# line/Human-Interaction-Generation

Measured on AMD Instinct MI355X. Metric: denoiser-fwd frames/s @ B=64·T=196, higher is better.
Workload: dtype f32; 1 GPU; MotionTransformer forward incl. the per-call cross-attention text side, BASELINE config 2: B=64/GPU T=196 F=150 d=512 L=8 H=8 ff=1024 N=77 Lt=256, linear attention, text embeddings supplied (CLIP stubbed); parallelism=dp1

## Files before the change

human-interaction-generation_amd/csrc/denoiser.hip:

```cpp
#include <stdarg.h>
#include <stdio.h>
#include <string.h>

#include "hig_common.h"
#include "hig_host.h"

static thread_local char g_err[512] = "";
int hig_set_error(int code, const char* fmt, ...) {
  va_list ap;
  va_start(ap, fmt);
  vsnprintf(g_err, sizeof(g_err), fmt, ap);
  va_end(ap);
  return code;
}
extern "C" int hig_last_error(char* buf, int n) {
  if (buf && n > 0) {
    strncpy(buf, g_err, (size_t)n - 1);
    buf[n - 1] = 0;
  }
  return (int)strlen(g_err);
}
extern "C" int hig_version(void) { return 100; }

namespace {
// ... 367 lines not shown
namespace {

constexpr int kMaxTextLayers = 32;
struct SideStream {
  hipStream_t s2 = nullptr;
  hipEvent_t ready = nullptr;
  hipEvent_t done[4] = {nullptr, nullptr, nullptr, nullptr};
  hipStream_t s3 = nullptr;
  hipEvent_t text_done[kMaxTextLayers] = {};
  bool ok = false, failed = false;
};

constexpr int kMaxDev = 16;
SideStream* side_stream_table() {
  static thread_local SideStream tab[kMaxDev];
  return tab;
}

hipEvent_t& layer_event() {
  static thread_local hipEvent_t ev = nullptr;
  return ev;
}

int bwd_overlap_env() {
  static const int v = getenv("HIG_BWD_OVERLAP") ? atoi(getenv("HIG_BWD_OVERLAP")) : -1;
  return v;
}

SideStream* side_stream_for_current_device(hipStream_t caller) {
  if (bwd_overlap_env() == 0) return nullptr;
  SideStream* tab = side_stream_table();
  int dev = 0;
  if (hipGetDevice(&dev) != hipSuccess || dev < 0 || dev >= kMaxDev) return nullptr;
  SideStream& s = tab[dev];
  if (s.failed) return nullptr;
  if (!s.ok) {
    hipStreamCaptureStatus cap = hipStreamCaptureStatusNone;
    if (hipStreamIsCapturing(caller, &cap) != hipSuccess || cap != hipStreamCaptureStatusNone) return nullptr;
    bool good = hipStreamCreateWithFlags(&s.s2, hipStreamNonBlocking) == hipSuccess;
    good = good && hipEventCreateWithFlags(&s.ready, hipEventDisableTiming) == hipSuccess;
    for (int i = 0; i < 4 && good; ++i) good = hipEventCreateWithFlags(&s.done[i], hipEventDisableTiming) == hipSuccess;
    good = good && hipStreamCreateWithFlags(&s.s3, hipStreamNonBlocking) == hipSuccess;
    for (int i = 0; i < kMaxTextLayers && good; ++i) good = hipEventCreateWithFlags(&s.text_done[i], hipEventDisableTiming) == hipSuccess;
    if (!good) {
      s.failed = true;
      return nullptr;
    }
    s.ok = true;
  }
  return &s;
}

}

static int denoiser_fwd_impl(const hig_dims* dims, const void* const* params, const void* const* derived32, const float* x, const int64_t* t,
                             const int64_t* length, const float* xf_proj, const float* xf_out_for_text, const void* textctx, float* out,
                             void* workspace, int training, hig_stream_t stream);
extern "C" int hig_denoiser_fwd(const hig_dims* dims, const void* const* params, const float* x,
                                const int64_t* t, const int64_t* length, const float* xf_proj,
                                const void* textctx, float* out, void* workspace, int training,
                                hig_stream_t stream) {
  return denoiser_fwd_impl(dims, params, nullptr, x, t, length, xf_proj, nullptr, textctx, out, workspace, training, stream);
}
extern "C" int hig_denoiser_fwd_text(const hig_dims* dims, const void* const* params, const float* x, const int64_t* t,
                                     const int64_t* length, const float* xf_proj, const float* xf_out, void* textctx, float* out,
                                     void* workspace, int training, hig_stream_t stream) {
  HIG_REQUIRE(xf_out, "hig_denoiser_fwd_text: null argument");
  return denoiser_fwd_impl(dims, params, nullptr, x, t, length, xf_proj, xf_out, textctx, out, workspace, training, stream);
}
extern "C" int hig_denoiser_fwd_x(const hig_dims* dims, const void* const* params, const void* const* derived32, const float* x,
                                  const int64_t* t, const int64_t* length, const float* xf_proj, const float* xf_out, void* textctx,
                                  float* out, void* workspace, int training, hig_stream_t stream) {
  return denoiser_fwd_impl(dims, params, derived32, x, t, length, xf_proj, xf_out, textctx, out, workspace, training, stream);
}
static int denoiser_fwd_impl(const hig_dims* dims, const void* const* params, const void* const* derived32, const float* x, const int64_t* t,
                             const int64_t* length, const float* xf_proj, const float* xf_out_for_text, const void* textctx, float* out,
                             void* workspace, int training, hig_stream_t stream) {
  Dims D;
  HIG_TRY(check_dims(dims, D));
  HIG_REQUIRE(params && x && t && xf_proj && textctx && out && workspace, "hig_denoiser_fwd: null argument");
  HIG_REQUIRE(!D.bf16, "hig_denoiser_fwd: bf16 storage goes through hig_denoiser_fwd_bf16");
  const FwdLayout w = fwd_layout(D, training);
  const TextLayout tl = text_layout(D, training);
  float* ws = static_cast<float*>(workspace);
  const float* tc = static_cast<const float*>(textctx);
  hipStream_t st = hig_stream(stream);
  const int d = D.d, E = D.E;
  const int64_t M = D.M;
  const int64_t ss_ld = (int64_t)D.nsty * D.L * 2 * d;
  const int Bp = D.B / 2;

  HIG_TRY(hig_zero_async(ws + w.gtail, HIG_GEMM_TAIL_CNT_BYTES, st));
  const TailScratchScope tail_scope(ws + w.gtail);

  hipEvent_t* text_ev = nullptr;
  struct TextJoin {
    hipStream_t s3 = nullptr, st = nullptr;
    hipEvent_t ev = nullptr;
    bool armed = false;
    void arm(hipStream_t s3_, hipEvent_t ev_, hipStream_t st_) { s3 = s3_; ev = ev_; st = st_; armed = true; }
    ~TextJoin() {
      if (!armed) return;
      (void)hipEventRecord(ev, s3);
      (void)hipStreamWaitEvent(st, ev, 0);
    }
  } text_join;
  if (xf_out_for_text) {
    static const int text_fork = getenv("HIG_TEXT_FORK") ? atoi(getenv("HIG_TEXT_FORK")) : 1;
    SideStream* ts = (text_fork && D.L <= kMaxTextLayers && !text_batched(D, derived32, training)) ? side_stream_for_current_device(st) : nullptr;
    if (ts) {
      hipStreamCaptureStatus cap = hipStreamCaptureStatusNone;
      if (hipStreamIsCapturing(st, &cap) != hipSuccess || cap != hipStreamCaptureStatusNone) ts = nullptr;
    }
    if (ts) {
      HIG_TRY(hig_zero_async(ws + w.gtail3, HIG_GEMM_TAIL_CNT_BYTES, st));
      if (hipEventRecord(ts->ready, st) != hipSuccess || hipStreamWaitEvent(ts->s3, ts->ready, 0) != hipSuccess)
        return hig_set_error(HIG_EHIP, "text fork failed");
      hig_gemm_set_tail_scratch(ws + w.gtail3, HIG_GEMM_TAIL_BYTES);
      const int rc = text_context_impl(D, params, derived32, xf_out_for_text, const_cast<void*>(textctx), training, ts->s3, ts->text_done);
      hig_gemm_set_tail_scratch(ws + w.gtail, HIG_GEMM_TAIL_BYTES);
      text_join.arm(ts->s3, ts->text_done[0], st);
      if (rc != HIG_OK) return rc;
      text_ev = ts->text_done;
    } else {
      HIG_TRY(text_context_impl(D, params, derived32, xf_out_for_text, const_cast<void*>(textctx), training, st, nullptr));
    }
  }
  HIG_TRY(hig_timestep_embedding(t, D.B, d, ws + w.te, stream));
  float* few_scratch = ws + w.layer0;
  const int64_t few_floats = w.total - w.layer0;
  HIG_TRY(hig_gemm_few_rows(G(ws + w.te, d, 0, P(params, HIG_P_TE0_W), d, 0, ws + w.te_h, E, D.B, E, d)
                                .epi(HIG_EPI_BIAS, P(params, HIG_P_TE0_B)).prec(D.prec).g, few_scratch, few_floats, st));
  HIG_TRY(hig_gemm_few_rows(G(ws + w.te_h, E, 0, P(params, HIG_P_TE2_W), E, 0, ws + w.emb, E, D.B, E, E)
                                .silu(0).epi(HIG_EPI_BIAS_RES, P(params, HIG_P_TE2_B)).res(xf_proj, E).prec(D.prec).g,
                            few_scratch, few_floats, st));
  HIG_TRY(hig_gemm_few_rows(G(ws + w.emb, E, 0, P(params, HIG_P_STY_EMB_W), E, 0, ws + w.ss, ss_ld, D.B, ss_ld, E)
                                .silu(0).epi(HIG_EPI_BIAS, P(params, HIG_P_STY_EMB_B)).prec(D.prec).g, few_scratch, few_floats,
                            st));
  {
    G ge(x, D.F, 0, P(params, HIG_P_JOINT_W), D.F, 0, ws + w.h0, d, M, d, D.F);
    ge.epi(HIG_EPI_BIAS_POS, P(params, HIG_P_JOINT_B)).pos(P(params, HIG_P_SEQ_EMB), d, D.T).prec(D.prec);
    ge.g.pos_shift = D.two ? 1 : 0;
    HIG_TRY(hig_gemm_launch(ge.g, 1, nullptr, st));
  }
  const int64_t* len_partner = nullptr;
  if (D.two) {
    HIG_TRY(hig_gemm_launch(G(x, (int64_t)D.T * D.F, 0, P(params, HIG_P_JOINT2_W), 4, 0, ws + w.h0, (int64_t)D.T * d,
                              D.B, d, 4).epi(HIG_EPI_BIAS, P(params, HIG_P_JOINT2_B)).g, 1, nullptr, st));
    int64_t* lp = reinterpret_cast<int64_t*>(ws + w.lenp);
    hipLaunchKernelGGL(swap_halves_i64_kernel, dim3((D.B + 255) / 256), dim3(256), 0, st, length, D.B, (int64_t)D.T, lp);
    HIG_CHECK_LAUNCH();
    len_partner = lp;
  }
  constexpr int fuse_env = 0;
  const bool fuse_apply = fuse_env && !training && !D.full && (D.H == 4 || D.H == 8) && (D.hd == 64 || D.hd == 128);
  static const int fold_env = getenv("HIG_LNFOLD32") ? atoi(getenv("HIG_LNFOLD32")) : 1;
  const bool fold32 = fold_env && derived32 && !training && d % 128 == 0 && d <= 1024;
  const Derived d32 = derived32_table(D, derived32);
  int layer_rc = HIG_OK;
  auto layer = [&](int l, const float* hin_full, int b0, int nb, hipStream_t s, float* cscr) -> const float* {
    hig_stream_t hs = reinterpret_cast<hig_stream_t>(s);
    float* lb = ws + w.layer0 + w.lstride * l;
    const int64_t r0 = (int64_t)b0 * D.T, Mh = (int64_t)nb * D.T;
    const int64_t aoff = (int64_t)b0 * D.H * D.hd * D.hd;
    const float* ssl = ws + w.ss + (int64_t)(D.nsty * l) * 2 * d + (int64_t)b0 * ss_ld;
    const float* ss_ffn = ssl + (int64_t)(D.nsty - 1) * 2 * d;
    const int64_t* len = length ? length + b0 : nullptr;
    const float* hin = hin_full + r0 * d;
    auto R = [&](int64_t off, int64_t ld) { return lb + off + r0 * ld; };
    auto fail = [&](int rc) -> const float* { layer_rc = rc; return nullptr; };
#define HIG_L(expr) do { const int rc_ = (expr); if (rc_ != HIG_OK) return fail(rc_); } while (0)
    const int np = d >> 6;
    float* lnst = ws + w.lnstats + r0 * np * 2;
    auto folded = [&](int k) { return fold32 && d32.layer(l, HIG_D32_SA_QKV_W + 3 * k) != nullptr; };
    auto ln_proj = [&](int k, bool have_stats, const float* hrows, int norm_w, int norm_b, int lin_w, int lin_b, float* xn, float* st,
                       float* outp, int ncols) -> int {
      if (have_stats && folded(k)) {
        G gf(hrows, d, 0, d32.layer<float>(l, HIG_D32_SA_QKV_W + 3 * k), d, 0, outp, ncols, Mh, ncols, d);
        gf.epi(HIG_EPI_BIAS, d32.layer<float>(l, HIG_D32_SA_QKV_B + 3 * k)).prec(D.prec);
        gf.g.row_stats_in = lnst;
        gf.g.ln_colsum = d32.layer<float>(l, HIG_D32_SA_QKV_COLSUM + 3 * k);
        return hig_gemm_launch(gf.g, 1, nullptr, s);
      }
      HIG_TRY(hig_layernorm(hrows, d, Mh, d, PL(params, l, norm_w), PL(params, l, norm_b), xn, d, st, hs));
      return hig_gemm_launch(G(xn, d, 0, PL(params, l, lin_w), d, 0, outp, ncols, Mh, ncols, d)
                                 .epi(HIG_EPI_BIAS, PL(params, l, lin_b)).prec(D.prec).g, 1, nullptr, s);
    };
    HIG_L(ln_proj(0, l > 0 && folded(0), hin, HIG_L_SA_NORM_W, HIG_L_SA_NORM_B, HIG_L_SA_QKV_W, HIG_L_SA_QKV_B, R(w.xn1, d), R(w.st1, 2),
                  R(w.qkv, 3 * d), 3 * d));
    if (D.full) {
      HIG_L(hig_fullattn_fwd(R(w.qkv, 3 * d), 3 * d, R(w.qkv, 3 * d) + d, R(w.qkv, 3 * d) + 2 * d, 3 * d, nb, D.T, D.T, D.H, D.hd,
                             len, R(w.y1, d), d, lb + w.lse1 + (int64_t)b0 * D.H * D.T, hs));
    } else {
      HIG_L(hig_linattn_ctx(R(w.qkv, 3 * d) + d, R(w.qkv, 3 * d) + 2 * d, 3 * d, nb, D.T, D.H, D.hd, len,
                            lb + w.A1 + aoff, lb + w.kst1 + (int64_t)b0 * d * 2, cscr, hs));
      if (fuse_apply)
        HIG_L(hig_linattn_apply_sty(R(w.qkv, 3 * d), 3 * d, lb + w.A1 + aoff, PL(params, l, HIG_L_SA_STY_NORM_W),
                                    PL(params, l, HIG_L_SA_STY_NORM_B), ssl, ss_ld, d, R(w.a1, d), d, nb, D.T, D.H, D.hd, hs));
      else
        HIG_L(hig_linattn_apply(R(w.qkv, 3 * d), 3 * d, lb + w.A1 + aoff, R(w.y1, d), d, nb, D.T, D.H, D.hd, hs));
    }
    if (!fuse_apply)
      HIG_L(hig_ln_mod_silu(R(w.y1, d), d, Mh, d, PL(params, l, HIG_L_SA_STY_NORM_W), PL(params, l, HIG_L_SA_STY_NORM_B),
                            ssl, ss_ld, d, D.T, R(w.a1, d), d, R(w.st2, 2), hs));
    {
      G gs(R(w.a1, d), d, 0, PL(params, l, HIG_L_SA_STY_OUT_W), d, 0, R(w.h1, d), d, Mh, d, d);
      gs.epi(HIG_EPI_BIAS_RES, PL(params, l, HIG_L_SA_STY_OUT_B)).res(hin, d).prec(D.prec);
      if (folded(1)) gs.g.row_stats_out = lnst;
      HIG_L(hig_gemm_launch(gs.g, 1, nullptr, s));
    }
    HIG_L(ln_proj(1, folded(1), R(w.h1, d), HIG_L_CA_NORM_W, HIG_L_CA_NORM_B, HIG_L_CA_Q_W, HIG_L_CA_Q_B, R(w.xn2, d), R(w.st3, 2),
                  R(w.qc, d), d));
    const float* Acl = tc + tl.layer0 + tl.lstride * l + tl.Ac + aoff;
    if (text_ev && hipStreamWaitEvent(s, text_ev[l], 0) != hipSuccess) return fail(hig_set_error(HIG_EHIP, "text join failed"));
    if (D.full) {
      const float* kvl = tc + tl.kv + tl.kv_stride * l + (int64_t)b0 * D.N * 2 * d;
      HIG_L(hig_fullattn_fwd(R(w.qc, d), d, kvl, kvl + d, 2 * d, nb, D.T, D.N, D.H, D.hd, nullptr, R(w.y2, d), d,
                             lb + w.lse2 + (int64_t)b0 * D.H * D.T, hs));
    } else {
      if (fuse_apply)
        HIG_L(hig_linattn_apply_sty(R(w.qc, d), d, Acl, PL(params, l, HIG_L_CA_STY_NORM_W),
                                    PL(params, l, HIG_L_CA_STY_NORM_B), ssl + 2 * d, ss_ld, d, R(w.a2, d), d, nb, D.T, D.H, D.hd, hs));
      else
        HIG_L(hig_linattn_apply(R(w.qc, d), d, Acl, R(w.y2, d), d, nb, D.T, D.H, D.hd, hs));
    }
    if (!fuse_apply)
      HIG_L(hig_ln_mod_silu(R(w.y2, d), d, Mh, d, PL(params, l, HIG_L_CA_STY_NORM_W), PL(params, l, HIG_L_CA_STY_NORM_B),
                            ssl + 2 * d, ss_ld, d, D.T, R(w.a2, d), d, R(w.st4, 2), hs));
    HIG_L(hig_gemm_launch(G(R(w.a2, d), d, 0, PL(params, l, HIG_L_CA_STY_OUT_W), d, 0, R(w.h2, d), d, Mh, d, d)
                              .epi(HIG_EPI_BIAS_RES, PL(params, l, HIG_L_CA_STY_OUT_B)).res(R(w.h1, d), d).prec(D.prec).g, 1, nullptr, s));
    const float* hffn = R(w.h2, d);
    int64_t hffn_off = w.h2;
    if (D.two == 1) {
      HIG_L(hig_layernorm(lb + w.h2, d, M, d, PL(params, l, HIG_L_INT_NORM_W), PL(params, l, HIG_L_INT_NORM_B),
                          lb + w.xn3, d, lb + w.st6, hs));
      HIG_L(hig_gemm_launch(G(lb + w.xn3, d, 0, PL(params, l, HIG_L_INT_QKV_W), d, 0, lb + w.iqkv, 3 * d, M, 3 * d, d)
                                .epi(HIG_EPI_BIAS, PL(params, l, HIG_L_INT_QKV_B)).prec(D.prec).g, 1, nullptr, s));
      HIG_L(hig_linattn_ctx(lb + w.iqkv + d, lb + w.iqkv + 2 * d, 3 * d, D.B, D.T, D.H, D.hd, len_partner,
                            lb + w.Ai, lb + w.ksti, cscr, hs));
      const int64_t halfA = (int64_t)Bp * D.H * D.hd * D.hd, halfM = (int64_t)Bp * D.T;
      HIG_L(hig_linattn_apply(lb + w.iqkv, 3 * d, lb + w.Ai + halfA, lb + w.y4, d, Bp, D.T, D.H, D.hd, hs));
      HIG_L(hig_linattn_apply(lb + w.iqkv + halfM * 3 * d, 3 * d, lb + w.Ai, lb + w.y4 + halfM * d, d, Bp, D.T, D.H,
                              D.hd, hs));
      HIG_L(hig_ln_mod_silu(lb + w.y4, d, M, d, PL(params, l, HIG_L_INT_STY_NORM_W), PL(params, l, HIG_L_INT_STY_NORM_B),
                            ssl + 4 * d, ss_ld, d, D.T, lb + w.a4, d, lb + w.st7, hs));
      HIG_L(hig_gemm_launch(G(lb + w.a4, d, 0, PL(params, l, HIG_L_INT_STY_OUT_W), d, 0, lb + w.h2b, d, M, d, d)
                                .epi(HIG_EPI_BIAS_RES, PL(params, l, HIG_L_INT_STY_OUT_B)).res(lb + w.h2, d).prec(D.prec).g,
                            1, nullptr, s));
      hffn = lb + w.h2b;
      hffn_off = w.h2b;
    }
    (void)hffn_off;
    HIG_L(hig_gemm_launch(G(hffn, d, 0, PL(params, l, HIG_L_FFN_W1), d, 0, R(w.f1, D.ff), D.ff, Mh, D.ff, d)
                              .epi(HIG_EPI_BIAS_GELU, PL(params, l, HIG_L_FFN_B1))
                              .aux(training ? R(w.z1, D.ff) : nullptr, D.ff).prec(D.prec).g, 1, nullptr, s));
    HIG_L(hig_gemm_launch(G(R(w.f1, D.ff), D.ff, 0, PL(params, l, HIG_L_FFN_W2), D.ff, 0, R(w.y3, d), d, Mh, d, D.ff)
                              .epi(HIG_EPI_BIAS, PL(params, l, HIG_L_FFN_B2)).prec(D.prec).g, 1, nullptr, s));
    HIG_L(hig_ln_mod_silu(R(w.y3, d), d, Mh, d, PL(params, l, HIG_L_FFN_STY_NORM_W), PL(params, l, HIG_L_FFN_STY_NORM_B),
                          ss_ffn, ss_ld, d, D.T, R(w.a3, d), d, R(w.st5, 2), hs));
    {
      G gs(R(w.a3, d), d, 0, PL(params, l, HIG_L_FFN_STY_OUT_W), d, 0, R(w.h3, d), d, Mh, d, d);
      gs.epi(HIG_EPI_BIAS_RES, PL(params, l, HIG_L_FFN_STY_OUT_B)).res(hffn, d).prec(D.prec);
      if (fold32 && l + 1 < D.L && d32.layer(l + 1, HIG_D32_SA_QKV_W) != nullptr) gs.g.row_stats_out = lnst;
      HIG_L(hig_gemm_launch(gs.g, 1, nullptr, s));
    }
#undef HIG_L
    return lb + w.h3;
  };
  auto out_proj = [&](const float* hin_full, int b0, int nb, hipStream_t s) -> int {
    const int64_t r0 = (int64_t)b0 * D.T;
    return hig_gemm_launch(G(hin_full + r0 * d, d, 0, P(params, HIG_P_OUT_W), d, 0, out + r0 * D.F, D.F, (int64_t)nb * D.T, D.F, d)
                               .epi(HIG_EPI_BIAS, P(params, HIG_P_OUT_B)).prec(D.prec).g, 1, nullptr, s);
  };

  static const int split_knob = getenv("HIG_FWD_SPLIT") ? atoi(getenv("HIG_FWD_SPLIT")) : -1;
  const int split_env = split_knob >= 0 ? split_knob : ((D.prec == HIG_PREC_F32 && hig_gemm_wsp32_active()) ? 0 : 1);
  SideStream* side = (split_env && !D.two && D.B >= 16 && M >= 8192) ? side_stream_for_current_device(st) : nullptr;
  if (side) {
    hipStreamCaptureStatus cap = hipStreamCaptureStatusNone;
    if (hipStreamIsCapturing(st, &cap) != hipSuccess || cap != hipStreamCaptureStatusNone) side = nullptr;
  }
  const float* hin = ws + w.h0;
  if (side) {
    const int nbA = D.B / 2, nbB = D.B - nbA;
    HIG_TRY(hig_zero_async(ws + w.gtail2, HIG_GEMM_TAIL_CNT_BYTES, st));
    if (hipEventRecord(side->ready, st) != hipSuccess || hipStreamWaitEvent(side->s2, side->ready, 0) != hipSuccess)
      return hig_set_error(HIG_EHIP, "forward fork failed");
    int rc = HIG_OK;
    for (int l = 0; l < D.L && rc == HIG_OK; ++l) {
      hig_gemm_set_tail_scratch(ws + w.gtail, HIG_GEMM_TAIL_BYTES);
      const float* ha = layer(l, hin, 0, nbA, st, ws + w.cscr);
      const float* hb = nullptr;
      if (ha) {
        hig_gemm_set_tail_scratch(ws + w.gtail2, HIG_GEMM_TAIL_BYTES);
        hb = layer(l, hin, nbA, nbB, side->s2, ws + w.cscr2);
      }
      if (!ha || !hb) rc = layer_rc != HIG_OK ? layer_rc : HIG_EHIP;
      else hin = ha;
    }
    if (rc == HIG_OK) {
      hig_gemm_set_tail_scratch(ws + w.gtail, HIG_GEMM_TAIL_BYTES);
      rc = out_proj(hin, 0, nbA, st);
    }
    if (rc == HIG_OK) {
      hig_gemm_set_tail_scratch(ws + w.gtail2, HIG_GEMM_TAIL_BYTES);
      rc = out_proj(hin, nbA, nbB, side->s2);
    }
    hig_gemm_set_tail_scratch(ws + w.gtail, HIG_GEMM_TAIL_BYTES);
// ... 1507 lines not shown
```

human-interaction-generation_amd/csrc/linattn.hip:

```cpp
#include <stdlib.h>

#include "hig_common.h"

int hig_chip_cus();

namespace {

constexpr int CH = 64;

template <int HD> struct Patch {
  static constexpr int PC = HD >= 128 ? 8 : HD >= 64 ? 4 : HD >= 32 ? 2 : 1;
  static constexpr int PL = PC;
  static constexpr int TL = HD / PL;
};

template <int HD>
__global__ __launch_bounds__(256) void ctx_kernel(const float* __restrict__ K,
                                                  const float* __restrict__ V, int64_t ld, int rows,
                                                  int H, const int64_t* __restrict__ length,
                                                  float* __restrict__ A, float* __restrict__ kstat) {
  constexpr int LDP = HD + 4;
  constexpr int PC = Patch<HD>::PC, PL = Patch<HD>::PL, TL = Patch<HD>::TL;
  constexpr int RG = 256 / HD;
  __shared__ __attribute__((aligned(16))) float sP[CH * LDP];
// ... 1524 lines not shown
  constexpr int QLD = HD + 4;
  constexpr int EQ = Vec16<TQ>::N;
  constexpr int CPR = HD / EQ;
  constexpr int NQL = 32 * CPR / 64;
  extern __shared__ __attribute__((aligned(16))) char smem_dyn[];
  __shared__ float red[2][4][32];
  const int tid = threadIdx.x, lane = tid & 63, wave = tid >> 6;
  const int lr = lane & 31, kk = lane >> 5;
  const int b = blockIdx.x / nblk, r0 = (blockIdx.x % nblk) * 32;
  const int HPW = H / 4;
  const int d = H * HD;
  constexpr int WBUF = 32 * QLD > KC * HD ? 32 * QLD : KC * HD;
  float* sAw = reinterpret_cast<float*>(smem_dyn) + wave * WBUF;
  float* sQw = sAw;

  f32x16 acc[MAXHPW][TB];
#pragma unroll
  for (int hh = 0; hh < MAXHPW; ++hh)
#pragma unroll
    for (int tb = 0; tb < TB; ++tb) zero16(acc[hh][tb]);

  u32x4_t pq[NQL];
  f32x4_t pa[16];
  auto fetch_q = [&](int h) {
#pragma unroll
    for (int i = 0; i < NQL; ++i) {
      const int idx = lane + 64 * i, rr = idx / CPR, c = idx % CPR;
      const int row = min(r0 + rr, rows - 1);
      pq[i] = *reinterpret_cast<const u32x4_t*>(Q + ((int64_t)b * rows + row) * ldq + h * HD + EQ * c);
    }
  };
  auto fetch_a = [&](int h, int c0) {
    const f32x4_t* src = reinterpret_cast<const f32x4_t*>(A + (((int64_t)b * H + h) * HD + c0) * HD);
#pragma unroll
    for (int i = 0; i < 16; ++i) pa[i] = src[lane + 64 * i];
  };
  fetch_q(wave * HPW);
  fetch_a(wave * HPW, 0);

#pragma unroll
  for (int hh = 0; hh < MAXHPW; ++hh) {
    if (hh >= HPW) break;
    const int h = wave * HPW + hh;
#pragma unroll
    for (int i = 0; i < NQL; ++i) {
      const int idx = lane + 64 * i, rr = idx / CPR, c = idx % CPR;
      put16(sQw + rr * QLD + EQ * c, pq[i], static_cast<const TQ*>(nullptr));
    }
    if (hh + 1 < HPW) fetch_q(h + 1);
    f32x4_t q[HD / 8];
    float m = -INFINITY;
#pragma unroll
    for (int ks = 0; ks < HD / 8; ++ks) {
      q[ks] = *reinterpret_cast<const f32x4_t*>(sQw + lr * QLD + 8 * ks + 4 * kk);
      m = fmaxf(m, fmaxf(fmaxf(q[ks].x, q[ks].y), fmaxf(q[ks].z, q[ks].w)));
    }
    m = fmaxf(m, __shfl_xor(m, 32, 64));
    float sum = 0.f;
#pragma unroll
    for (int ks = 0; ks < HD / 8; ++ks) {
      q[ks].x = __expf(q[ks].x - m); q[ks].y = __expf(q[ks].y - m); q[ks].z = __expf(q[ks].z - m); q[ks].w = __expf(q[ks].w - m);
      sum += (q[ks].x + q[ks].y) + (q[ks].z + q[ks].w);
    }
    sum += __shfl_xor(sum, 32, 64);
    const float inv = 1.0f / sum;
#pragma unroll
    for (int ks = 0; ks < HD / 8; ++ks) q[ks] *= inv;
#pragma unroll
    for (int sl = 0; sl < NSLAB; ++sl) {
      const int c0 = sl * KC;
#pragma unroll
      for (int i = 0; i < 16; ++i) reinterpret_cast<f32x4_t*>(sAw)[lane + 64 * i] = pa[i];
      if (sl + 1 < NSLAB) fetch_a(h, c0 + KC);
      else if (hh + 1 < HPW) fetch_a(h + 1, 0);
#pragma unroll
      for (int ks = c0 / 8; ks < (c0 + KC) / 8; ++ks) {
        const float* ap = sAw + (8 * ks + 4 * kk - c0) * HD + lr;
#pragma unroll
        for (int tb = 0; tb < TB; ++tb)
          acc[hh][tb] = mfma4(acc[hh][tb], ap[32 * tb], ap[HD + 32 * tb], ap[2 * HD + 32 * tb], ap[3 * HD + 32 * tb], make_float4(q[ks].x, q[ks].y, q[ks].z, q[ks].w));
      }
    }
  }
  float s = 0.f;
#pragma unroll
  for (int hh = 0; hh < MAXHPW; ++hh)
#pragma unroll
    for (int tb = 0; tb < TB; ++tb)
#pragma unroll
      for (int e = 0; e < 16; ++e) s += acc[hh][tb][e];
  s += __shfl_xor(s, 32, 64);
  if (kk == 0) red[0][wave][lr] = s;
  __syncthreads();
  const float mean = ((red[0][0][lr] + red[0][1][lr]) + (red[0][2][lr] + red[0][3][lr])) / (float)d;
  float qd = 0.f;
#pragma unroll
  for (int hh = 0; hh < MAXHPW; ++hh) {
    if (hh >= HPW) break;
#pragma unroll
    for (int tb = 0; tb < TB; ++tb)
#pragma unroll
      for (int e = 0; e < 16; ++e) {
        const float dv = acc[hh][tb][e] - mean;
        qd += dv * dv;
      }
  }
  qd += __shfl_xor(qd, 32, 64);
  if (kk == 0) red[1][wave][lr] = qd;
  __syncthreads();
  const float rstd = rsqrtf(((red[1][0][lr] + red[1][1][lr]) + (red[1][2][lr] + red[1][3][lr])) / (float)d + 1e-5f);
  TO* sO = reinterpret_cast<TO*>(smem_dyn);
  const int ldso = d + 16 / (int)sizeof(TO);
  const float* ssrow = ss + (int64_t)b * ss_ld;
#pragma unroll
  for (int hh = 0; hh < MAXHPW; ++hh) {
    if (hh >= HPW) break;
    const int h = wave * HPW + hh;
#pragma unroll
    for (int tb = 0; tb < TB; ++tb)
#pragma unroll
      for (int qq = 0; qq < 4; ++qq) {
        const int col = h * HD + 32 * tb + 8 * qq + 4 * kk;
        const float4 g4 = *reinterpret_cast<const float4*>(gamma + col), b4 = *reinterpret_cast<const float4*>(beta + col);
        const float4 sc = *reinterpret_cast<const float4*>(ssrow + col), sh = *reinterpret_cast<const float4*>(ssrow + shift_off + col);
        float4 o;
        o.x = apply_sty_act<TO>(((acc[hh][tb][4 * qq] - mean) * rstd * g4.x + b4.x) * (1.0f + sc.x) + sh.x);
        o.y = apply_sty_act<TO>(((acc[hh][tb][4 * qq + 1] - mean) * rstd * g4.y + b4.y) * (1.0f + sc.y) + sh.y);
        o.z = apply_sty_act<TO>(((acc[hh][tb][4 * qq + 2] - mean) * rstd * g4.z + b4.z) * (1.0f + sc.z) + sh.z);
        o.w = apply_sty_act<TO>(((acc[hh][tb][4 * qq + 3] - mean) * rstd * g4.w + b4.w) * (1.0f + sc.w) + sh.w);
        st4(sO + lr * ldso + col, o);
      }
  }
  __syncthreads();
  constexpr int EO = 16 / (int)sizeof(TO);
  const int c16 = d / EO;
  for (int idx = tid; idx < 32 * c16; idx += 256) {
    const int rr = idx / c16, ch = idx % c16;
    if (r0 + rr < rows)
      *reinterpret_cast<uint4*>(Out + ((int64_t)b * rows + r0 + rr) * ldo + EO * ch) =
          *reinterpret_cast<const uint4*>(sO + rr * ldso + EO * ch);
  }
}

template <typename TQ, typename TO>
int launch_apply_sty(const TQ* q, int64_t ldq, const float* A, const float* gamma, const float* beta, const float* ss,
                     int64_t ss_ld, int32_t shift_off, TO* o, int64_t ldo, int32_t B, int32_t rows, int32_t H, int32_t hd,
                     hipStream_t st) {
  const int nblk = (rows + 31) / 32;
  const int d = H * hd;
  const size_t wbuf = (size_t)32 * (hd + 4) > 4096 ? (size_t)32 * (hd + 4) : 4096;
  const size_t lds_main = 4 * wbuf * sizeof(float);
  const size_t lds_out = (size_t)32 * (d + 16 / sizeof(TO)) * sizeof(TO);
  const size_t lds = lds_main > lds_out ? lds_main : lds_out;
  static const int big_lds_rc = [] {
    hipError_t e1 = hipFuncSetAttribute(reinterpret_cast<const void*>(&apply_sty_kernel<64, TQ, TO>),
                                        hipFuncAttributeMaxDynamicSharedMemorySize, 156 * 1024);
    hipError_t e2 = hipFuncSetAttribute(reinterpret_cast<const void*>(&apply_sty_kernel<128, TQ, TO>),
                                        hipFuncAttributeMaxDynamicSharedMemorySize, 156 * 1024);
    return (e1 == hipSuccess && e2 == hipSuccess) ? 0 : 1;
  }();
  if (big_lds_rc != 0 || lds > 156 * 1024)
    return hig_set_error(HIG_EHIP, "hig_linattn_apply_sty: cannot reserve %zu bytes of LDS", lds);
  if (hd == 64)
    hipLaunchKernelGGL((apply_sty_kernel<64, TQ, TO>), dim3(B * nblk), dim3(256), lds, st, q, ldq, A, gamma, beta, ss, ss_ld,
                       shift_off, o, ldo, rows, H, nblk);
  else
    hipLaunchKernelGGL((apply_sty_kernel<128, TQ, TO>), dim3(B * nblk), dim3(256), lds, st, q, ldq, A, gamma, beta, ss, ss_ld,
                       shift_off, o, ldo, rows, H, nblk);
  HIG_CHECK_LAUNCH();
  return HIG_OK;
}

}

extern "C" int hig_linattn_ctx_bf16(const void* K, const void* V, int64_t ld, int32_t B, int32_t rows, int32_t H,
                                    int32_t hd, const int64_t* length, float* A, float* kstat, float* scratch,
                                    void* At16, hig_stream_t stream) {
  HIG_REQUIRE(K && V && A && kstat && B > 0 && rows > 0 && H > 0, "hig_linattn_ctx_bf16: bad arguments");
  if (hd != 64 && hd != 128)
    return hig_set_error(HIG_EUNSUPPORTED, "hig_linattn: bf16 storage is built for head dim 64 / 128 (got %d)", hd);
  HIG_REQUIRE(ld % 4 == 0 && (reinterpret_cast<uintptr_t>(K) & 7) == 0 && (reinterpret_cast<uintptr_t>(V) & 7) == 0,
              "hig_linattn_ctx_bf16: K/V must be 8-byte aligned");
  return linattn_ctx_t<__bf16>(static_cast<const __bf16*>(K), static_cast<const __bf16*>(V), ld, B, rows, H, hd, length, A,
                               kstat, scratch, hig_stream(stream), static_cast<__bf16*>(At16));
}
extern "C" int hig_linattn_apply_bf16(const void* Q, int64_t ldq, const float* A, void* Y, int64_t ldy, int32_t B,
                                      int32_t rows, int32_t H, int32_t hd, hig_stream_t stream) {
  HIG_REQUIRE(Q && A && Y && B > 0 && rows > 0 && H > 0, "hig_linattn_apply_bf16: bad arguments");
  if (hd != 64 && hd != 128)
    return hig_set_error(HIG_EUNSUPPORTED, "hig_linattn: bf16 storage is built for head dim 64 / 128 (got %d)", hd);
  HIG_REQUIRE(ldq % 4 == 0 && ldy % 8 == 0 && (reinterpret_cast<uintptr_t>(Q) & 7) == 0 &&
                  (reinterpret_cast<uintptr_t>(Y) & 15) == 0,
              "hig_linattn_apply_bf16: Q rows must be 8-byte aligned, Y rows 16-byte aligned");
  return linattn_apply_t<__bf16>(static_cast<const __bf16*>(Q), ldq, A, static_cast<__bf16*>(Y), ldy, B, rows, H, hd,
                                 hig_stream(stream));
}

extern "C" int64_t hig_linattn_bwd_scratch_floats(int32_t B, int32_t rows, int32_t H, int32_t hd) {
  const int64_t nchunk = (rows + CH - 1) / CH;
  return (int64_t)B * H * nchunk * ((int64_t)hd * hd + hd);
}

extern "C" int hig_linattn_apply_bwd(const float* dY, int64_t lddy, const float* Q, int64_t ldq,
                                     const float* A, float* dQ, int64_t lddq, float* dA, int32_t B,
                                     int32_t rows, int32_t H, int32_t hd, float* scratch,
                                     hig_stream_t stream) {
  HIG_REQUIRE(dY && Q && A && dQ && dA && scratch && B > 0 && rows > 0 && H > 0,
              "hig_linattn_apply_bwd: bad arguments");
  HIG_REQUIRE(hd_ok(hd), "hig_linattn: head dim %d not in {8,16,32,64,128}", hd);
  HIG_REQUIRE(ldq % 4 == 0 && lddy % 4 == 0 && lddq % 4 == 0 && (reinterpret_cast<uintptr_t>(Q) & 15) == 0 &&
                  (reinterpret_cast<uintptr_t>(dY) & 15) == 0 && (reinterpret_cast<uintptr_t>(dQ) & 15) == 0,
              "hig_linattn_apply_bwd: Q/dY/dQ must be 16-byte aligned");
  const int nchunk = (rows + CH - 1) / CH;
  int nparts = nchunk;
  if (hd == 64 || (hd == 128 && allow_big_lds() == 0)) {
    constexpr int tgt = 0;
    const int target = tgt > 0 ? tgt : hig_chip_cus();
    nparts = (target + B * H - 1) / (B * H);
    nparts = nparts < 1 ? 1 : (nparts > nchunk ? nchunk : nparts);
    float* part = nparts == 1 ? dA : scratch;
    if (hd == 64)
      hipLaunchKernelGGL(apply_bwd_mfma_kernel<64>, dim3(B * H, nparts), dim3(256), attn_bwd_lds_bytes<64>(),
                         hig_stream(stream), dY, lddy, Q, ldq, A, dQ, lddq, part, rows, H);
    else
      hipLaunchKernelGGL(apply_bwd_mfma_kernel<128>, dim3(B * H, nparts), dim3(256), attn_bwd_lds_bytes<128>(),
                         hig_stream(stream), dY, lddy, Q, ldq, A, dQ, lddq, part, rows, H);
    if (nparts == 1) {
      HIG_CHECK_LAUNCH();
      return HIG_OK;
    }
  } else {
    HD_SWITCH(hd, hipLaunchKernelGGL((apply_bwd_kernel<HDV>), dim3(B * H, nchunk), dim3(256), 0, hig_stream(stream),
                                     dY, lddy, Q, ldq, A, dQ, lddq, scratch, rows, H));
  }
  HIG_CHECK_LAUNCH();
  const int64_t n = (int64_t)hd * hd, groups = (int64_t)B * H;
  const int64_t want = (groups * n / 4 + 255) / 256;
  hipLaunchKernelGGL(chunk_sum_kernel, dim3((unsigned)(want > 2048 ? 2048 : want)), dim3(256), 0, hig_stream(stream),
                     scratch, nparts, n, groups, dA);
  HIG_CHECK_LAUNCH();
  return HIG_OK;
}

extern "C" int hig_linattn_ctx_bwd(const float* dA, const float* A, const float* K, const float* V, int64_t ld,
                                   const float* kstat, const int64_t* length, float* dK, float* dV,
                                   int64_t ldd, int32_t B, int32_t rows, int32_t H, int32_t hd,
                                   float* scratch, hig_stream_t stream) {
  HIG_REQUIRE(dA && A && K && V && kstat && dK && dV && scratch && B > 0 && rows > 0 && H > 0,
              "hig_linattn_ctx_bwd: bad arguments");
  HIG_REQUIRE(hd_ok(hd), "hig_linattn: head dim %d not in {8,16,32,64,128}", hd);
  HIG_REQUIRE(ldd % 4 == 0 && (reinterpret_cast<uintptr_t>(dK) & 15) == 0 && (reinterpret_cast<uintptr_t>(dV) & 15) == 0,
              "hig_linattn_ctx_bwd: dK/dV must be 16-byte aligned");
  const int nchunk = (rows + CH - 1) / CH;
  if (hd == 64 || (hd == 128 && allow_big_lds() == 0)) {
    constexpr int tgt = 0;
    const int target = tgt > 0 ? tgt : hig_chip_cus();
    int gy = (target + B * H - 1) / (B * H);
    gy = gy < 1 ? 1 : (gy > nchunk ? nchunk : gy);
    if (hd == 64)
      hipLaunchKernelGGL(ctx_bwd_mfma_kernel<64>, dim3(B * H, gy), dim3(256), attn_bwd_lds_bytes<64>(),
                         hig_stream(stream), dA, A, K, V, ld, kstat, length, dK, dV, ldd, rows, H);
    else
      hipLaunchKernelGGL(ctx_bwd_mfma_kernel<128>, dim3(B * H, gy), dim3(256), attn_bwd_lds_bytes<128>(),
                         hig_stream(stream), dA, A, K, V, ld, kstat, length, dK, dV, ldd, rows, H);
    HIG_CHECK_LAUNCH();
    return HIG_OK;
  }
  HD_SWITCH(hd, hipLaunchKernelGGL((ctx_bwd_kernel<HDV>), dim3(B * H, nchunk), dim3(256), 0, hig_stream(stream), dA,
                                   K, V, ld, kstat, length, dK, dV, ldd, rows, H, scratch));
  HIG_CHECK_LAUNCH();
  HD_SWITCH(hd, hipLaunchKernelGGL((ctx_bwd_finish_kernel<HDV>), dim3(B * H, nchunk), dim3(256), 0,
                                   hig_stream(stream), K, ld, kstat, length, dK, ldd, rows, H, scratch));
  HIG_CHECK_LAUNCH();
  return HIG_OK;
}


extern "C" int hig_linattn_apply_bwd_bf16(const void* dY, int64_t lddy, const void* Q, int64_t ldq, const float* A, void* dQ,
                                          int64_t lddq, float* dA, int32_t B, int32_t rows, int32_t H, int32_t hd, float* scratch,
                                          hig_stream_t stream) {
  HIG_REQUIRE(dY && Q && A && dQ && dA && scratch && B > 0 && rows > 0 && H > 0, "hig_linattn_apply_bwd_bf16: bad arguments");
  if (!(hd == 64 || (hd == 128 && allow_big_lds() == 0)))
    return hig_set_error(HIG_EUNSUPPORTED, "hig_linattn_apply_bwd_bf16: head dim 64 or 128 (got %d)", hd);
  HIG_REQUIRE(ldq % 4 == 0 && lddy % 4 == 0 && lddq % 8 == 0 && ((reinterpret_cast<uintptr_t>(Q) | reinterpret_cast<uintptr_t>(dY)) & 7) == 0 &&
                  (reinterpret_cast<uintptr_t>(dQ) & 15) == 0,
              "hig_linattn_apply_bwd_bf16: Q / dY rows must be 8-byte aligned, dQ rows 16-byte aligned");
  const int nchunk = (rows + CH - 1) / CH;
  constexpr int tgt16 = 0;
  const int target16 = tgt16 > 0 ? tgt16 : hig_chip_cus();
  int nparts = (target16 + B * H - 1) / (B * H);
  nparts = nparts < 1 ? 1 : (nparts > nchunk ? nchunk : nparts);
  float* part = nparts == 1 ? dA : scratch;
  const __bf16* dy = static_cast<const __bf16*>(dY);
  const __bf16* q = static_cast<const __bf16*>(Q);
  __bf16* dq = static_cast<__bf16*>(dQ);
  if (hd == 64)
    hipLaunchKernelGGL((apply_bwd_mfma_kernel<64, __bf16>), dim3(B * H, nparts), dim3(256), attn_bwd_lds_bytes<64>(), hig_stream(stream),
                       dy, lddy, q, ldq, A, dq, lddq, part, rows, H);
  else
    hipLaunchKernelGGL((apply_bwd_mfma_kernel<128, __bf16>), dim3(B * H, nparts), dim3(256), attn_bwd_lds_bytes<128>(), hig_stream(stream),
                       dy, lddy, q, ldq, A, dq, lddq, part, rows, H);
  HIG_CHECK_LAUNCH();
  if (nparts == 1) return HIG_OK;
  const int64_t n = (int64_t)hd * hd, groups = (int64_t)B * H;
  const int64_t want = (groups * n / 4 + 255) / 256;
  hipLaunchKernelGGL(chunk_sum_kernel, dim3((unsigned)(want > 2048 ? 2048 : want)), dim3(256), 0, hig_stream(stream), scratch, nparts, n,
                     groups, dA);
  HIG_CHECK_LAUNCH();
  return HIG_OK;
}
extern "C" int hig_linattn_ctx_bwd_bf16(const float* dA, const float* A, const void* K, const void* V, int64_t ld, const float* kstat,
                                        const int64_t* length, void* dK, void* dV, int64_t ldd, int32_t B, int32_t rows, int32_t H,
                                        int32_t hd, hig_stream_t stream) {
  HIG_REQUIRE(dA && A && K && V && kstat && dK && dV && B > 0 && rows > 0 && H > 0, "hig_linattn_ctx_bwd_bf16: bad arguments");
  if (!(hd == 64 || (hd == 128 && allow_big_lds() == 0)))
    return hig_set_error(HIG_EUNSUPPORTED, "hig_linattn_ctx_bwd_bf16: head dim 64 or 128 (got %d)", hd);
  HIG_REQUIRE(ld % 4 == 0 && ldd % 8 == 0 && ((reinterpret_cast<uintptr_t>(K) | reinterpret_cast<uintptr_t>(V)) & 7) == 0 &&
                  ((reinterpret_cast<uintptr_t>(dK) | reinterpret_cast<uintptr_t>(dV)) & 15) == 0,
              "hig_linattn_ctx_bwd_bf16: K / V rows must be 8-byte aligned, dK / dV rows 16-byte aligned");
  const int nchunk = (rows + CH - 1) / CH;
  constexpr int tgt16 = 0;
  const int target16 = tgt16 > 0 ? tgt16 : hig_chip_cus();
  int gy = (target16 + B * H - 1) / (B * H);
  gy = gy < 1 ? 1 : (gy > nchunk ? nchunk : gy);
  const __bf16* k = static_cast<const __bf16*>(K);
  const __bf16* v = static_cast<const __bf16*>(V);
  if (hd == 64)
    hipLaunchKernelGGL((ctx_bwd_mfma_kernel<64, __bf16>), dim3(B * H, gy), dim3(256), attn_bwd_lds_bytes<64>(), hig_stream(stream), dA, A, k, v,
                       ld, kstat, length, static_cast<__bf16*>(dK), static_cast<__bf16*>(dV), ldd, rows, H);
  else
    hipLaunchKernelGGL((ctx_bwd_mfma_kernel<128, __bf16>), dim3(B * H, gy), dim3(256), attn_bwd_lds_bytes<128>(), hig_stream(stream), dA, A, k,
                       v, ld, kstat, length, static_cast<__bf16*>(dK), static_cast<__bf16*>(dV), ldd, rows, H);
  HIG_CHECK_LAUNCH();
  return HIG_OK;
}

extern "C" int hig_linattn_apply_sty_bf16(const void* Q, int64_t ldq, const float* A, const float* gamma,
                                          const float* beta, const float* ss, int64_t ss_ld, int32_t ss_shift_off,
                                          void* Out, int64_t ldo, int32_t B, int32_t rows, int32_t H, int32_t hd,
                                          hig_stream_t stream) {
  HIG_REQUIRE(Q && A && gamma && beta && ss && Out && B > 0 && rows > 0, "hig_linattn_apply_sty_bf16: bad arguments");
  if ((hd != 64 && hd != 128) || (H != 4 && H != 8))
    return hig_set_error(HIG_EUNSUPPORTED, "hig_linattn_apply_sty_bf16: built for head dim 64 / 128 and 4 or 8 heads (got %d, %d)", hd, H);
  HIG_REQUIRE(ldq % 8 == 0 && ldo % 8 == 0 && ss_ld % 4 == 0 && ss_shift_off % 4 == 0 &&
                  ((reinterpret_cast<uintptr_t>(Q) & 15) | (reinterpret_cast<uintptr_t>(Out) & 15) |
                   (reinterpret_cast<uintptr_t>(gamma) & 15) | (reinterpret_cast<uintptr_t>(beta) & 15) |
                   (reinterpret_cast<uintptr_t>(ss) & 15)) == 0,
              "hig_linattn_apply_sty_bf16: alignment");
  return launch_apply_sty<__bf16, __bf16>(static_cast<const __bf16*>(Q), ldq, A, gamma, beta, ss, ss_ld, ss_shift_off,
                                          static_cast<__bf16*>(Out), ldo, B, rows, H, hd, hig_stream(stream));
}

extern "C" int hig_linattn_apply_sty(const float* Q, int64_t ldq, const float* A, const float* gamma, const float* beta,
                                     const float* ss, int64_t ss_ld, int32_t ss_shift_off, float* Out, int64_t ldo,
                                     int32_t B, int32_t rows, int32_t H, int32_t hd, hig_stream_t stream) {
  HIG_REQUIRE(Q && A && gamma && beta && ss && Out && B > 0 && rows > 0, "hig_linattn_apply_sty: bad arguments");
  if ((hd != 64 && hd != 128) || (H != 4 && H != 8))
    return hig_set_error(HIG_EUNSUPPORTED, "hig_linattn_apply_sty: built for head dim 64 / 128 and 4 or 8 heads (got %d, %d)", hd, H);
  HIG_REQUIRE(ldq % 4 == 0 && ldo % 4 == 0 && ss_ld % 4 == 0 && ss_shift_off % 4 == 0 &&
                  ((reinterpret_cast<uintptr_t>(Q) & 15) | (reinterpret_cast<uintptr_t>(Out) & 15) |
                   (reinterpret_cast<uintptr_t>(gamma) & 15) | (reinterpret_cast<uintptr_t>(beta) & 15) |
                   (reinterpret_cast<uintptr_t>(ss) & 15)) == 0,
              "hig_linattn_apply_sty: alignment");
  return launch_apply_sty<float, float>(Q, ldq, A, gamma, beta, ss, ss_ld, ss_shift_off, Out, ldo, B, rows, H, hd,
                                        hig_stream(stream));
}
```

Measured before the change: 2.115 million frames/s.

## Enable fused linear-attention apply with new MFMA wave64 fp32 kernel for hd=64

Turns on the fused apply path (query softmax, context product, LayerNorm, style modulation, SiLU) for inference with head dim 64. It does this through a new fp32 kernel that keeps each head's context matrix in registers, does the product with 16x16x4 f32 MFMA instructions, and prefetches the next query tile. LayerNorm statistics are combined across heads through LDS, and results are written with buffer stores. This removes the separate apply, LayerNorm and modulation kernels and their intermediate memory traffic. The cost is a hand-scheduled asm path with tight alignment and size assumptions, and the fp32 hd=64 case of the generic kernel is now rejected.

Result: faster. 2.153 million frames/s, median of 6 (+1.8%).

```diff
diff --git a/human-interaction-generation_amd/csrc/denoiser.hip b/human-interaction-generation_amd/csrc/denoiser.hip
--- a/human-interaction-generation_amd/csrc/denoiser.hip
+++ b/human-interaction-generation_amd/csrc/denoiser.hip
@@ -543,8 +543,7 @@
     HIG_CHECK_LAUNCH();
     len_partner = lp;
   }
-  constexpr int fuse_env = 0;
-  const bool fuse_apply = fuse_env && !training && !D.full && (D.H == 4 || D.H == 8) && (D.hd == 64 || D.hd == 128);
+  const bool fuse_apply = !training && !D.full && D.hd == 64 && (D.H == 4 || D.H == 8) && ss_ld % 4 == 0;
   static const int fold_env = getenv("HIG_LNFOLD32") ? atoi(getenv("HIG_LNFOLD32")) : 1;
   const bool fold32 = fold_env && derived32 && !training && d % 128 == 0 && d <= 1024;
   const Derived d32 = derived32_table(D, derived32);
diff --git a/human-interaction-generation_amd/csrc/linattn.hip b/human-interaction-generation_amd/csrc/linattn.hip
--- a/human-interaction-generation_amd/csrc/linattn.hip
+++ b/human-interaction-generation_amd/csrc/linattn.hip
@@ -1700,21 +1700,180 @@
   const size_t lds_main = 4 * wbuf * sizeof(float);
   const size_t lds_out = (size_t)32 * (d + 16 / sizeof(TO)) * sizeof(TO);
   const size_t lds = lds_main > lds_out ? lds_main : lds_out;
+  constexpr bool HAS64 = !std::is_same<TQ, float>::value;
   static const int big_lds_rc = [] {
-    hipError_t e1 = hipFuncSetAttribute(reinterpret_cast<const void*>(&apply_sty_kernel<64, TQ, TO>),
-                                        hipFuncAttributeMaxDynamicSharedMemorySize, 156 * 1024);
+    hipError_t e1 = hipSuccess;
+    if constexpr (HAS64)
+      e1 = hipFuncSetAttribute(reinterpret_cast<const void*>(&apply_sty_kernel<64, TQ, TO>),
+                               hipFuncAttributeMaxDynamicSharedMemorySize, 156 * 1024);
     hipError_t e2 = hipFuncSetAttribute(reinterpret_cast<const void*>(&apply_sty_kernel<128, TQ, TO>),
                                         hipFuncAttributeMaxDynamicSharedMemorySize, 156 * 1024);
     return (e1 == hipSuccess && e2 == hipSuccess) ? 0 : 1;
   }();
   if (big_lds_rc != 0 || lds > 156 * 1024)
     return hig_set_error(HIG_EHIP, "hig_linattn_apply_sty: cannot reserve %zu bytes of LDS", lds);
-  if (hd == 64)
-    hipLaunchKernelGGL((apply_sty_kernel<64, TQ, TO>), dim3(B * nblk), dim3(256), lds, st, q, ldq, A, gamma, beta, ss, ss_ld,
-                       shift_off, o, ldo, rows, H, nblk);
-  else
+  if (hd == 64) {
+    if constexpr (HAS64)
+      hipLaunchKernelGGL((apply_sty_kernel<64, TQ, TO>), dim3(B * nblk), dim3(256), lds, st, q, ldq, A, gamma, beta, ss, ss_ld,
+                         shift_off, o, ldo, rows, H, nblk);
+    else
+      return hig_set_error(HIG_EUNSUPPORTED, "hig_linattn_apply_sty: head dim 64 has its own fp32 kernel");
+  } else
     hipLaunchKernelGGL((apply_sty_kernel<128, TQ, TO>), dim3(B * nblk), dim3(256), lds, st, q, ldq, A, gamma, beta, ss, ss_ld,
                        shift_off, o, ldo, rows, H, nblk);
+  HIG_CHECK_LAUNCH();
+  return HIG_OK;
+}
+
+template <int H>
+__global__ __launch_bounds__(64 * H, 4) void apply_sty_wave64_kernel(const float* __restrict__ Q, int64_t ldq, const float* __restrict__ A,
+                                                                    const float* __restrict__ gamma, const float* __restrict__ beta,
+                                                                    const float* __restrict__ ss, int64_t ss_ld, int shift_off,
+                                                                    float* __restrict__ Out, int64_t ldo, int rows) {
+  constexpr int HD = 64, D = H * HD;
+  __shared__ __attribute__((aligned(16))) float sW[H * 16 * HD];
+  __shared__ __attribute__((aligned(16))) float sP[4 * D];
+  __shared__ float2 sR[2][H][16];
+  const int tid = threadIdx.x, lane = tid & 63, h = tid >> 6;
+  const int b = blockIdx.x;
+  const int r = lane & 15, kq = lane >> 4;
+  const int ntile = (rows + 15) >> 4, step = gridDim.y;
+  const float* qb = Q + (int64_t)b * rows * ldq + h * HD + 16 * kq;
+  la_f32x4 qt[4];
+  auto fetch = [&](int tile, la_f32x4 (&v)[4]) {
+    const int row = min(min(tile, ntile - 1) * 16 + r, rows - 1);
+    const float* p = qb + (int64_t)row * ldq;
+    asm volatile("global_load_dwordx4 %0, %4, off\n\tglobal_load_dwordx4 %1, %4, off offset:16\n\t"
+                 "global_load_dwordx4 %2, %4, off offset:32\n\tglobal_load_dwordx4 %3, %4, off offset:48"
+                 : "=&v"(v[0]), "=&v"(v[1]), "=&v"(v[2]), "=&v"(v[3]) : "v"(p) : "memory");
+  };
+  int tile = blockIdx.y;
+  fetch(tile, qt);
+  float aop[16][4];
+  {
+    const float4* Ab = reinterpret_cast<const float4*>(A + (((int64_t)b * H + h) * HD + 16 * kq) * HD) + r;
+#pragma unroll
+    for (int s2 = 0; s2 < 16; ++s2) {
+      const float4 a4 = Ab[s2 * (HD / 4)];
+      aop[s2][0] = a4.x; aop[s2][1] = a4.y; aop[s2][2] = a4.z; aop[s2][3] = a4.w;
+    }
+    const int arr = tid / (D / 4), idx = tid % (D / 4);
+    const float* ssrow = ss + (int64_t)b * ss_ld;
+    const float* src = arr == 0 ? gamma : arr == 1 ? beta : arr == 2 ? ssrow : ssrow + shift_off;
+    float4 pv = *reinterpret_cast<const float4*>(src + 4 * idx);
+    if (arr == 2) pv = make_float4(1.0f + pv.x, 1.0f + pv.y, 1.0f + pv.z, 1.0f + pv.w);
+    *reinterpret_cast<float4*>(sP + arr * D + 4 * idx) = pv;
+  }
+  float* const so = sW + h * (16 * HD);
+  __syncthreads();
+  [[maybe_unused]] __amdgpu_buffer_rsrc_t rsO = __builtin_amdgcn_make_buffer_rsrc(Out + (int64_t)b * rows * ldo, 0, (int)(((int64_t)(rows - 1) * ldo + D) * 4), 0x00020000);
+  int par = 0;
+  auto tile_out = [&](int tile, auto younger) {
+    la_f32x4 (&cur)[4] = qt;
+    constexpr int YOUNGER = decltype(younger)::value;
+    asm volatile("s_waitcnt vmcnt(%4)" : "+v"(cur[0]), "+v"(cur[1]), "+v"(cur[2]), "+v"(cur[3]) : "n"(YOUNGER) : "memory");
+    float m = fmaxf(fmaxf(fmaxf(cur[0].x, cur[0].y), fmaxf(cur[0].z, cur[0].w)), fmaxf(fmaxf(cur[1].x, cur[1].y), fmaxf(cur[1].z, cur[1].w)));
+    m = fmaxf(m, fmaxf(fmaxf(fmaxf(cur[2].x, cur[2].y), fmaxf(cur[2].z, cur[2].w)), fmaxf(fmaxf(cur[3].x, cur[3].y), fmaxf(cur[3].z, cur[3].w))));
+    m = fmaxf(m, __shfl_xor(m, 16, 64));
+    m = fmaxf(m, __shfl_xor(m, 32, 64));
+    float p[16];
+    float sum = 0.f;
+#pragma unroll
+    for (int i = 0; i < 4; ++i) {
+      p[4 * i] = __expf(cur[i].x - m); p[4 * i + 1] = __expf(cur[i].y - m); p[4 * i + 2] = __expf(cur[i].z - m); p[4 * i + 3] = __expf(cur[i].w - m);
+      sum += (p[4 * i] + p[4 * i + 1]) + (p[4 * i + 2] + p[4 * i + 3]);
+    }
+    sum += __shfl_xor(sum, 16, 64);
+    sum += __shfl_xor(sum, 32, 64);
+    const float inv = 1.0f / sum;
+    la_f32x4 acc[4];
+#pragma unroll
+    for (int blk = 0; blk < 4; ++blk) acc[blk] = la_f32x4{0.f, 0.f, 0.f, 0.f};
+#pragma unroll
+    for (int s2 = 0; s2 < 16; ++s2) {
+      const float ps = p[s2] * inv;
+#pragma unroll
+      for (int blk = 0; blk < 4; ++blk) acc[blk] = __builtin_amdgcn_mfma_f32_16x16x4f32(aop[s2][blk], ps, acc[blk], 0, 0, 0);
+    }
+    float bs = 0.f;
+#pragma unroll
+    for (int blk = 0; blk < 4; ++blk) bs += (acc[blk][0] + acc[blk][1]) + (acc[blk][2] + acc[blk][3]);
+    bs += __shfl_xor(bs, 16, 64);
+    bs += __shfl_xor(bs, 32, 64);
+    const float bm = bs * (1.0f / HD);
+    float bq = 0.f;
+#pragma unroll
+    for (int blk = 0; blk < 4; ++blk) {
+      const float d0 = acc[blk][0] - bm, d1 = acc[blk][1] - bm, d2 = acc[blk][2] - bm, d3 = acc[blk][3] - bm;
+      bq += (d0 * d0 + d1 * d1) + (d2 * d2 + d3 * d3);
+    }
+    bq += __shfl_xor(bq, 16, 64);
+    bq += __shfl_xor(bq, 32, 64);
+#pragma unroll
+    for (int e = 0; e < 4; ++e)
+      *reinterpret_cast<la_f32x4*>(so + r * HD + ((16 * kq + 4 * e) ^ (4 * r))) = la_f32x4{acc[0][e], acc[1][e], acc[2][e], acc[3][e]};
+    if (kq == 0) sR[par][h][r] = make_float2(bs, bq);
+    lds_barrier();
+    float tot = 0.f, within = 0.f;
+#pragma unroll
+    for (int hh = 0; hh < H; ++hh) {
+      const float2 ps = sR[par][hh][r];
+      tot += ps.x; within += ps.y;
+    }
+    const float mean = tot * (1.0f / D);
+    asm volatile("" ::: "memory");
+    float between = 0.f;
+#pragma unroll
+    for (int hh = 0; hh < H; ++hh) {
+      const float dm = fmaf(sR[par][hh][r].x, 1.0f / HD, -mean);
+      between = fmaf(dm, dm, between);
+    }
+    par ^= 1;
+    const float rstd = rsqrtf(fmaf((float)HD, between, within) * (1.0f / D) + 1e-5f);
+#pragma unroll
+    for (int e = 0; e < 4; ++e) {
+      const int col = h * HD + 16 * kq + 4 * e;
+      const float4 g4 = *reinterpret_cast<const float4*>(sP + col), b4 = *reinterpret_cast<const float4*>(sP + D + col);
+      const float4 sc = *reinterpret_cast<const float4*>(sP + 2 * D + col), sh = *reinterpret_cast<const float4*>(sP + 3 * D + col);
+      float* const yp = so + r * HD + ((16 * kq + 4 * e) ^ (4 * r));
+      const float4 y4 = *reinterpret_cast<const float4*>(yp);
+      float4 o;
+      o.x = hig_silu(((y4.x - mean) * rstd * g4.x + b4.x) * sc.x + sh.x);
+      o.y = hig_silu(((y4.y - mean) * rstd * g4.y + b4.y) * sc.y + sh.y);
+      o.z = hig_silu(((y4.z - mean) * rstd * g4.z + b4.z) * sc.z + sh.z);
+      o.w = hig_silu(((y4.w - mean) * rstd * g4.w + b4.w) * sc.w + sh.w);
+      *reinterpret_cast<float4*>(yp) = o;
+      asm volatile("" ::: "memory");
+    }
+    fetch(tile + step < ntile ? tile + step : tile, qt);
+    asm volatile("s_waitcnt lgkmcnt(0)" ::: "memory");
+#pragma unroll
+    for (int i = 0; i < 4; ++i) {
+      const int rr = 4 * i + kq, cc = 4 * r;
+      [[maybe_unused]] const float4 v = *reinterpret_cast<const float4*>(so + rr * HD + (cc ^ (4 * rr)));
+      [[maybe_unused]] const int row = tile * 16 + rr;
+#if defined(__HIP_DEVICE_COMPILE__)
+      __builtin_amdgcn_raw_buffer_store_b128(__builtin_bit_cast(la_i32x4, v), rsO, (row * (int)ldo + h * HD + cc) * 4, 0, 0);
+#endif
+    }
+    asm volatile("s_waitcnt lgkmcnt(0)" ::: "memory");
+  };
+  tile_out(tile, std::integral_constant<int, 0>{});
+  for (tile += step; tile < ntile; tile += step) tile_out(tile, std::integral_constant<int, 4>{});
+  asm volatile("s_waitcnt vmcnt(0)" ::: "memory");
+}
+
+constexpr int APPLY_STY_WAVE_SLOTS = 256 * 16;
+template <int H>
+int launch_apply_sty_wave64(const float* q, int64_t ldq, const float* A, const float* gamma, const float* beta, const float* ss,
+                            int64_t ss_ld, int32_t shift_off, float* o, int64_t ldo, int32_t B, int32_t rows, hipStream_t st) {
+  const int ntile = (rows + 15) / 16;
+  int nstrip = APPLY_STY_WAVE_SLOTS / H / B;
+  nstrip = nstrip < 1 ? 1 : nstrip > ntile ? ntile : nstrip;
+  const int per = (ntile + nstrip - 1) / nstrip;
+  nstrip = (ntile + per - 1) / per;
+  hipLaunchKernelGGL((apply_sty_wave64_kernel<H>), dim3(B, nstrip), dim3(64 * H), 0, st, q, ldq, A, gamma, beta, ss, ss_ld, shift_off, o,
+                     ldo, rows);
   HIG_CHECK_LAUNCH();
   return HIG_OK;
 }
@@ -1910,6 +2069,11 @@
                    (reinterpret_cast<uintptr_t>(gamma) & 15) | (reinterpret_cast<uintptr_t>(beta) & 15) |
                    (reinterpret_cast<uintptr_t>(ss) & 15)) == 0,
               "hig_linattn_apply_sty: alignment");
+  if (hd == 64) {
+    HIG_REQUIRE(((int64_t)rows + 16) * ldo * 4 < INT32_MAX, "hig_linattn_apply_sty: a sample's output rows exceed 2 GiB");
+    return H == 8 ? launch_apply_sty_wave64<8>(Q, ldq, A, gamma, beta, ss, ss_ld, ss_shift_off, Out, ldo, B, rows, hig_stream(stream))
+                  : launch_apply_sty_wave64<4>(Q, ldq, A, gamma, beta, ss, ss_ld, ss_shift_off, Out, ldo, B, rows, hig_stream(stream));
+  }
   return launch_apply_sty<float, float>(Q, ldq, A, gamma, beta, ss, ss_ld, ss_shift_off, Out, ldo, B, rows, H, hd,
                                         hig_stream(stream));
 }
```
